# OpenMendel/MendelIHT.jl

Hardware: NVIDIA B200
Metric: iht_iterations_per_sec (higher is better)
Workload: dtype f64 (sweep: f32 LUT partials per slab of 640 samples (512 without the ternary copy), f64 across slabs; top-k candidates re-scored in f64)

## Files before the change

mendeliht.jl_b200/csrc/lut_common.cuh:

```cuda
#pragma once
#include "common.cuh"
#include <cuda_fp16.h>

namespace ihtb {

constexpr int LUT_TABLE_BYTES = 131072;

__device__ __forceinline__ uint32_t smem_u32(const void* p) { return (uint32_t)__cvta_generic_to_shared(p); }
__device__ __forceinline__ void mbar_init(uint32_t bar, uint32_t count) {
    asm volatile("mbarrier.init.shared::cta.b64 [%0], %1;" ::"r"(bar), "r"(count));
}
__device__ __forceinline__ void mbar_arrive(uint32_t bar) {
    asm volatile("mbarrier.arrive.shared::cta.b64 _, [%0];" ::"r"(bar) : "memory");
}
__device__ __forceinline__ void mbar_expect_tx(uint32_t bar, uint32_t bytes) {
    asm volatile("mbarrier.arrive.expect_tx.shared::cta.b64 _, [%0], %1;" ::"r"(bar), "r"(bytes) : "memory");
}
__device__ __forceinline__ void mbar_wait(uint32_t bar, uint32_t parity) {
    asm volatile(
        "{\n\t.reg .pred p;\n"
        "W_%=:\n\t"
        "mbarrier.try_wait.parity.shared::cta.b64 p, [%0], %1;\n\t"
        "@!p bra W_%=;\n\t}"
        ::"r"(bar), "r"(parity) : "memory");
}
__device__ __forceinline__ void bulk_g2s(uint32_t dst, const void* src, uint32_t bytes, uint32_t bar) {
    asm volatile("cp.async.bulk.shared::cluster.global.mbarrier::complete_tx::bytes [%0], [%1], %2, [%3];"
                 ::"r"(dst), "l"(src), "r"(bytes), "r"(bar) : "memory");
}
__device__ __forceinline__ float lds_f32(uint32_t addr) {
    float v;
    asm volatile("ld.shared.f32 %0, [%1];" : "=f"(v) : "r"(addr));
    return v;
}
__device__ __forceinline__ uint32_t lds_u32(uint32_t addr) {
    uint32_t v;
    asm volatile("ld.shared.u32 %0, [%1];" : "=r"(v) : "r"(addr));
    return v;
}
__device__ __forceinline__ uint4 lds_u128(uint32_t addr) {
    uint4 v;
    asm volatile("ld.shared.v4.u32 {%0, %1, %2, %3}, [%4];" : "=r"(v.x), "=r"(v.y), "=r"(v.z), "=r"(v.w) : "r"(addr));
    return v;
}
__device__ __forceinline__ void sts_u32(uint32_t addr, uint32_t v) {
    asm volatile("st.shared.u32 [%0], %1;" ::"r"(addr), "r"(v) : "memory");
}
__device__ __forceinline__ void sts_f32(uint32_t addr, float v) {
    asm volatile("st.shared.f32 [%0], %1;" ::"r"(addr), "f"(v) : "memory");
}
template <int NT>
__device__ __forceinline__ void consumer_bar() {
    asm volatile("bar.sync 1, %0;" ::"n"(NT) : "memory");
}

template <int NT>
__device__ __forceinline__ void lut_build(uint32_t tab, const double* __restrict__ v, double vbar, int64_t n,
                                          int64_t slab, int tid) {
    constexpr int PARTS = NT / 128;
    constexpr int V3_PER = 4 / PARTS;
    const int group = tid & 127, part = tid >> 7;
    const int t = group >> 5, w = group & 31;
    float u[4];
#pragma unroll
    for (int s = 0; s < 4; ++s) {
        int64_t i = slab * 512 + 16 * w + 4 * t + s;
        u[s] = (i < n) ? __double2float_rn(__dsub_rn(v[i], vbar)) : 0.0f;
    }
    auto f = [&](int s, int code) -> float { return code == 2 ? u[s] : (code == 3 ? u[s] + u[s] : 0.0f); };
    const uint32_t rowbase = tab + (uint32_t)(t >> 1) * 65536u + (uint32_t)(t & 1) * 128u + 4u * (uint32_t)w;
#pragma unroll
    for (int c3 = 0; c3 < V3_PER; ++c3) {
        const int v3 = part * V3_PER + c3;
        const float a3 = (v3 == 2) ? u[3] : ((v3 == 3) ? u[3] + u[3] : 0.0f);
        const uint32_t base3 = rowbase + (uint32_t)v3 * (64u * 256u);
#pragma unroll
        for (int v2 = 0; v2 < 4; ++v2) {
            const float a2 = a3 + f(2, v2);
#pragma unroll
            for (int v1 = 0; v1 < 4; ++v1) {
                const float a1 = a2 + f(1, v1);
#pragma unroll
                for (int v0 = 0; v0 < 4; ++v0)
                    sts_f32(base3 + (uint32_t)(v2 << 4 | v1 << 2 | v0) * 256u, a1 + f(0, v0));
            }
        }
    }
}

template <int NT>
__device__ __forceinline__ void lut_build_tern(uint32_t tab, const double* __restrict__ v, double vbar, int64_t n,
                                               int64_t slab, int tid) {
    static_assert(NT == 512, "ternary tables are built by 512 threads");
    const int group = tid & 127, d4 = tid >> 7;
    if (d4 > 2) return;
    const int t = group >> 5, w = group & 31;
    float u[5];
#pragma unroll
    for (int s = 0; s < 5; ++s) {
        int64_t i = slab * 640 + 20 * w + 5 * t + s;
        u[s] = (i < n) ? __double2float_rn(__dsub_rn(v[i], vbar)) : 0.0f;
    }
    auto f = [&](int s, int d) -> float { return d == 1 ? u[s] : (d == 2 ? u[s] + u[s] : 0.0f); };
    const uint32_t rowbase = tab + (uint32_t)(t >> 1) * 65536u + (uint32_t)(t & 1) * 128u + 4u * (uint32_t)w;
    const float a4 = (d4 == 1) ? u[4] : ((d4 == 2) ? u[4] + u[4] : 0.0f);
    const uint32_t base4 = rowbase + (uint32_t)d4 * (81u * 256u);
#pragma unroll
    for (int d3 = 0; d3 < 3; ++d3) {
        const float a3 = a4 + f(3, d3);
#pragma unroll
        for (int d2 = 0; d2 < 3; ++d2) {
            const float a2 = a3 + f(2, d2);
#pragma unroll
            for (int d1 = 0; d1 < 3; ++d1) {
                const float a1 = a2 + f(1, d1);
#pragma unroll
                for (int d0 = 0; d0 < 3; ++d0)
                    sts_f32(base4 + (uint32_t)(27 * d3 + 9 * d2 + 3 * d1 + d0) * 256u, a1 + f(0, d0));
            }
        }
    }
}

__device__ __forceinline__ void lut_build_h2_tern(uint32_t tab, const double* __restrict__ v0, const double* __restrict__ v1,
                                                  double vbar0, double vbar1, float sc0, float sc1, int64_t n, int64_t slab,
                                                  int tid) {
    const int group = tid & 127, d4 = tid >> 7;
    if (d4 > 2) return;
    const int t = group >> 5, w = group & 31;
    float a[5], b[5];
#pragma unroll
    for (int s = 0; s < 5; ++s) {
        int64_t i = slab * 640 + 20 * w + 5 * t + s;
        const float x0 = (i < n) ? __double2float_rn(__dsub_rn(v0[i], vbar0)) * sc0 : 0.0f;
        const float x1 = (i < n) ? __double2float_rn(__dsub_rn(v1[i], vbar1)) * sc1 : 0.0f;
        a[s] = (w & 16) ? x1 : x0;
        b[s] = (w & 16) ? x0 : x1;
    }
    auto fa = [&](int s, int d) -> float { return d == 1 ? a[s] : (d == 2 ? a[s] + a[s] : 0.0f); };
    auto fb = [&](int s, int d) -> float { return d == 1 ? b[s] : (d == 2 ? b[s] + b[s] : 0.0f); };
    const uint32_t rowbase = tab + (uint32_t)(t >> 1) * 65536u + (uint32_t)(t & 1) * 128u + 4u * (uint32_t)w;
    const float a4 = fa(4, d4), b4 = fb(4, d4);
    const uint32_t base4 = rowbase + (uint32_t)d4 * (81u * 256u);
#pragma unroll
    for (int d3 = 0; d3 < 3; ++d3) {
        const float a3 = a4 + fa(3, d3), b3 = b4 + fb(3, d3);
#pragma unroll
        for (int d2 = 0; d2 < 3; ++d2) {
            const float a2 = a3 + fa(2, d2), b2 = b3 + fb(2, d2);
#pragma unroll
            for (int d1 = 0; d1 < 3; ++d1) {
                const float a1 = a2 + fa(1, d1), b1 = b2 + fb(1, d1);
#pragma unroll
                for (int d0 = 0; d0 < 3; ++d0) {
                    const __half2 h = __floats2half2_rn(a1 + fa(0, d0), b1 + fb(0, d0));
                    sts_u32(base4 + (uint32_t)(27 * d3 + 9 * d2 + 3 * d1 + d0) * 256u, *reinterpret_cast<const uint32_t*>(&h));
                }
            }
        }
    }
}

__device__ __forceinline__ void lut_build_h2(uint32_t tab, const double* __restrict__ v0, const double* __restrict__ v1,
                                             double vbar0, double vbar1, float sc0, float sc1, int64_t n, int64_t slab,
                                             int tid) {
    const int group = tid & 127, part = tid >> 7;
    const int t = group >> 5, w = group & 31;
    float a[4], b[4];
#pragma unroll
    for (int s = 0; s < 4; ++s) {
        int64_t i = slab * 512 + 16 * w + 4 * t + s;
        a[s] = (i < n) ? __double2float_rn(__dsub_rn(v0[i], vbar0)) * sc0 : 0.0f;
        b[s] = (i < n) ? __double2float_rn(__dsub_rn(v1[i], vbar1)) * sc1 : 0.0f;
    }
    auto fa = [&](int s, int code) -> float { return code == 2 ? a[s] : (code == 3 ? a[s] + a[s] : 0.0f); };
    auto fb = [&](int s, int code) -> float { return code == 2 ? b[s] : (code == 3 ? b[s] + b[s] : 0.0f); };
    const uint32_t rowbase = tab + (uint32_t)(t >> 1) * 65536u + (uint32_t)(t & 1) * 128u + 4u * (uint32_t)w;
    const int v3 = part;
    const float a3 = fa(3, v3), b3 = fb(3, v3);
    const uint32_t base3 = rowbase + (uint32_t)v3 * (64u * 256u);
#pragma unroll
    for (int v2 = 0; v2 < 4; ++v2) {
        const float a2 = a3 + fa(2, v2), b2 = b3 + fb(2, v2);
#pragma unroll
        for (int v1c = 0; v1c < 4; ++v1c) {
            const float a1 = a2 + fa(1, v1c), b1 = b2 + fb(1, v1c);
#pragma unroll
            for (int v0c = 0; v0c < 4; ++v0c) {
                const __half2 h = __floats2half2_rn(a1 + fa(0, v0c), b1 + fb(0, v0c));
                sts_u32(base3 + (uint32_t)(v2 << 4 | v1c << 2 | v0c) * 256u, *reinterpret_cast<const uint32_t*>(&h));
            }
        }
    }
}

}
```

mendeliht.jl_b200/csrc/sweep_lut.cu:

```cuda
#include "lut_common.cuh"
#include <stdlib.h>

namespace ihtb {

constexpr int LUT_STAGE_COLS = 128;
constexpr int LUT_STAGE_BYTES = LUT_STAGE_COLS * 128;
constexpr int LUT_MAX_STAGES = 8;
constexpr int LUT_SMEM_BYTES = 232448;

struct LutPlan {
    uint32_t bar_full, bar_empty;
    uint32_t tab;
    uint32_t lo0, hi0;
    int n_lo, n_stages;
    __device__ __forceinline__ uint32_t stage(int s) const {
        return (s < n_lo) ? lo0 + (uint32_t)s * LUT_STAGE_BYTES : hi0 + (uint32_t)(s - n_lo) * LUT_STAGE_BYTES;
    }
};
__device__ __forceinline__ LutPlan lut_plan(uint32_t base, uint32_t bytes) {
    LutPlan pl;
    uint32_t end = base + bytes;
    pl.tab = (base + 65535u) & ~65535u;
    pl.bar_full = 0; pl.bar_empty = 0; pl.n_stages = 0;
    uint32_t lo = (base + 127u) & ~127u, lo_end = pl.tab;
    uint32_t hi = pl.tab + LUT_TABLE_BYTES, hi_end = end;
    if (lo + 256u <= lo_end) { pl.bar_full = lo; lo += 256u; }
    else { pl.bar_full = hi; hi += 256u; }
    pl.bar_empty = pl.bar_full + 8u * 2u * LUT_MAX_STAGES;
    pl.lo0 = lo; pl.hi0 = hi;
    pl.n_lo = (lo_end > lo) ? (int)((lo_end - lo) / LUT_STAGE_BYTES) : 0;
    if (pl.n_lo > LUT_MAX_STAGES) pl.n_lo = LUT_MAX_STAGES;
    int n_hi = (hi_end > hi) ? (int)((hi_end - hi) / LUT_STAGE_BYTES) : 0;
    pl.n_stages = pl.n_lo + n_hi;
    if (pl.n_stages > LUT_MAX_STAGES) pl.n_stages = LUT_MAX_STAGES;
    return pl;
}

template <int CW, int G, bool QUAD, bool H2, bool TERN>
__global__ void __launch_bounds__((CW + 1) * 32, 1)
k_sweep_lut(const uint8_t* __restrict__ bed, int64_t cs_j, int64_t cs_s, int64_t p, int64_t p_out, int64_t n,
            int64_t n_slabs, const double* __restrict__ v, const double* __restrict__ v1,
            const double* __restrict__ vbar_p, const float* __restrict__ scale_p, float* __restrict__ part,
            uint32_t dyn_bytes) {
    const double vbar = vbar_p[0];
    const double vbar1 = H2 ? vbar_p[1] : 0.0;
    const float sc0 = H2 ? scale_p[0] : 1.0f, sc1 = H2 ? scale_p[1] : 1.0f;
    constexpr int WPG = CW / G;
    constexpr int CPW = LUT_STAGE_COLS / WPG;
    static_assert(!QUAD || CPW % 4 == 0, "quad layout: a warp owns whole quads");
    static_assert(!H2 || (CW == 16 && CPW == 16), "pair sweep: 512 table builders, 16 columns per warp");
    static_assert(!TERN || (QUAD && CPW == 16), "ternary tiles: quad layout, 16 columns per warp");
    extern __shared__ __align__(128) uint8_t smem_raw[];
    const LutPlan pl = lut_plan(smem_u32(smem_raw), dyn_bytes);
    const int warp = threadIdx.x >> 5, lane = threadIdx.x & 31;
    const int S = pl.n_stages;
    const int period = (S % G == 0) ? S : S * G;

    const int64_t n_cblocks = (p + LUT_STAGE_COLS - 1) / LUT_STAGE_COLS;
    const int64_t units = n_slabs * n_cblocks;
    const int64_t u_beg = units * (int64_t)blockIdx.x / gridDim.x;
    const int64_t u_end = units * (int64_t)(blockIdx.x + 1) / gridDim.x;
    if (u_beg >= u_end) return;
    const int64_t slab_beg = u_beg / n_cblocks, slab_end = (u_end - 1) / n_cblocks;
    const int ncb = (int)n_cblocks;

    if (threadIdx.x == 0) {
        for (int s = 0; s < S; ++s) {
            for (int g = 0; g < G; ++g) mbar_init(pl.bar_full + 8u * (g * LUT_MAX_STAGES + s), 1);
            mbar_init(pl.bar_empty + 8u * s, WPG);
        }
        asm volatile("fence.mbarrier_init.release.cluster;" ::: "memory");
    }
    __syncthreads();

    if (warp == CW) {
        int st = 0; uint32_t ph = 0;
        int grp_of = 0;
        for (int64_t slab = slab_beg; slab <= slab_end; ++slab) {
            const int cb0 = (slab == slab_beg) ? (int)(u_beg - slab * n_cblocks) : 0;
            const int cb1 = (slab == slab_end) ? (int)(u_end - slab * n_cblocks) : ncb;
            for (int cb = cb0; cb < cb1; ++cb) {
                const int64_t j0 = (int64_t)cb * LUT_STAGE_COLS;
                const int ncols = (int)((p - j0 < LUT_STAGE_COLS) ? (p - j0) : LUT_STAGE_COLS);
                const uint32_t fullbar = pl.bar_full + 8u * (uint32_t)(grp_of * LUT_MAX_STAGES + st);
                mbar_wait(pl.bar_empty + 8u * st, ph ^ 1u);
                const uint8_t* src = bed + j0 * cs_j + slab * cs_s;
                if (cs_j == 128) {
                    if (lane == 0) {
                        mbar_expect_tx(fullbar, (uint32_t)ncols * 128u);
                        bulk_g2s(pl.stage(st), src, (uint32_t)ncols * 128u, fullbar);
                    }
                } else {
                    if (lane == 0) mbar_expect_tx(fullbar, (uint32_t)ncols * 128u);
                    __syncwarp();
                    for (int c = lane; c < ncols; c += 32)
                        bulk_g2s(pl.stage(st) + 128u * c, src + (int64_t)c * cs_j, 128u, fullbar);
                }
                if (++st == S) { st = 0; ph ^= 1u; }
                if (++grp_of == G) grp_of = 0;
            }
        }
    } else {
        const int tid = threadIdx.x;
        const int grp = warp / WPG, wg = warp % WPG;
        uint32_t lb[4];
#pragma unroll
        for (int t = 0; t < 4; ++t)
            lb[t] = pl.tab + (uint32_t)(t >> 1) * 65536u + (uint32_t)(t & 1) * 128u + 4u * (uint32_t)lane;
        constexpr int NACC = H2 ? 2 * CPW : CPW;
        constexpr int LPC = 32 / NACC > 0 ? 32 / NACC : 1;
        const int vidx = TERN ? (lane & (NACC - 1)) : lane / LPC;
        const int col = wg * CPW + vidx % CPW;
        const bool writer = TERN ? (lane < NACC) : (lane & (LPC - 1)) == 0;
        const uint32_t lqs = TERN ? ((((uint32_t)lane >> 2) & 3u) << 9) : 0u;
        const uint32_t lane_off = (uint32_t)(wg * CPW) * 128u + (QUAD ? 16u : 4u) * (uint32_t)lane;
        int st = grp % S, ip = grp % period; uint32_t ph = (uint32_t)((grp / period) & 1);
        const uint32_t my_full = pl.bar_full + 8u * (uint32_t)(grp * LUT_MAX_STAGES);
        int i_next = grp;
        int i_base = 0;
        for (int64_t slab = slab_beg; slab <= slab_end; ++slab) {
            const int cb0 = (slab == slab_beg) ? (int)(u_beg - slab * n_cblocks) : 0;
            const int cb1 = (slab == slab_end) ? (int)(u_end - slab * n_cblocks) : ncb;
            consumer_bar<CW * 32>();
            if (H2 && TERN) lut_build_h2_tern(pl.tab, v, v1, vbar, vbar1, sc0, sc1, n, slab, tid);
            else if (H2) lut_build_h2(pl.tab, v, v1, vbar, vbar1, sc0, sc1, n, slab, tid);
            else if (TERN) lut_build_tern<CW * 32>(pl.tab, v, vbar, n, slab, tid);
            else lut_build<CW * 32>(pl.tab, v, vbar, n, slab, tid);
            consumer_bar<CW * 32>();
            float* __restrict__ outp = part + ((int64_t)(H2 ? vidx / CPW : 0) * n_slabs + slab) * p_out + col;
            const int i_end = i_base + (cb1 - cb0);
            for (; i_next < i_end; i_next += G) {
                const int cb = cb0 + (i_next - i_base);
                mbar_wait(my_full + 8u * st, ph);
                const uint32_t colbase = pl.stage(st) + lane_off;
                float acc[NACC];
                uint4 q4 = make_uint4(0u, 0u, 0u, 0u);
#pragma unroll
                for (int c = 0; c < CPW; ++c) {
                    uint32_t w;
                    if (QUAD) {
                        if ((c & 3) == 0) q4 = lds_u128(colbase + ((512u * (c >> 2)) ^ lqs));
                        w = (c & 3) == 0 ? q4.x : (c & 3) == 1 ? q4.y : (c & 3) == 2 ? q4.z : q4.w;
                    } else {
                        w = lds_u32(colbase + 128u * c);
                    }
                    if (!H2) {
                        const float t0 = lds_f32(__byte_perm(w, lb[0], 0x7604));
                        const float t1 = lds_f32(__byte_perm(w, lb[1], 0x7614));
                        const float t2 = lds_f32(__byte_perm(w, lb[2], 0x7624));
                        const float t3 = lds_f32(__byte_perm(w, lb[3], 0x7634));
                        acc[c] = (t0 + t1) + (t2 + t3);
                    } else {
                        const uint32_t r0 = lds_u32(__byte_perm(w, lb[0], 0x7604));
                        const uint32_t r1 = lds_u32(__byte_perm(w, lb[1], 0x7614));
                        const uint32_t r2 = lds_u32(__byte_perm(w, lb[2], 0x7624));
                        const uint32_t r3 = lds_u32(__byte_perm(w, lb[3], 0x7634));
                        const __half2 h = __hadd2(__hadd2(*reinterpret_cast<const __half2*>(&r0), *reinterpret_cast<const __half2*>(&r1)),
                                                  __hadd2(*reinterpret_cast<const __half2*>(&r2), *reinterpret_cast<const __half2*>(&r3)));
                        const float2 f = __half22float2(h);
                        acc[c] = f.x;
                        acc[(H2 ? CPW : 0) + c] = f.y;
                    }
                }
                __syncwarp();
                if (lane == 0) mbar_arrive(pl.bar_empty + 8u * st);
                if (TERN) {
                    int o = NACC / 2;
#pragma unroll
                    for (int h = NACC / 2; h >= 1; h >>= 1, o >>= 1) {
#pragma unroll
                        for (int c = 0; c < h; ++c) acc[c] = acc[c] + __shfl_xor_sync(0xffffffffu, acc[c + h], o);
                    }
#pragma unroll
                    for (int oo = 16; oo >= NACC; oo >>= 1) acc[0] += __shfl_xor_sync(0xffffffffu, acc[0], oo);
                } else {
                    int o = 16;
#pragma unroll
                    for (int h = NACC / 2; h >= 1; h >>= 1, o >>= 1) {
                        const bool upper = (lane & o) != 0;
#pragma unroll
                        for (int c = 0; c < h; ++c) {
                            const float send = upper ? acc[c] : acc[c + h];
                            const float keep = upper ? acc[c + h] : acc[c];
                            acc[c] = keep + __shfl_xor_sync(0xffffffffu, send, o);
                        }
                    }
#pragma unroll
                    for (int oo = 16 / NACC; oo >= 1; oo >>= 1) acc[0] += __shfl_xor_sync(0xffffffffu, acc[0], oo);
                }
                const int jj = cb * LUT_STAGE_COLS + col;
                if (writer && jj < (int)p_out) outp[cb * LUT_STAGE_COLS] = acc[0];
                st += G; if (st >= S) st -= S;
                ip += G; if (ip >= period) { ip -= period; ph ^= 1u; }
            }
            i_base = i_end;
        }
    }
}

bool sweep_tmem_enabled(const ihtb_geno* g);
bool sweep_uses_tern(const ihtb_geno* g) { return g->tern.p != nullptr && g->quad && !sweep_tmem_enabled(g); }
int64_t sweep_fast_num_slabs(const ihtb_geno* g) { return sweep_uses_tern(g) ? g->tern_slabs : g->stride / 128; }

bool sweep_tmem_enabled(const ihtb_geno* g);
void sweep_tmem_partials(const ihtb_geno* g, const double* d_v, const double* d_vbar, float* d_part, cudaStream_t s);
void sweep_tmem_pair_partials(const ihtb_geno* g, const double* d_v0, const double* d_v1, const double* d_vbar,
                              const float* d_scale, float* d_part, cudaStream_t s);

template <bool QUAD, bool H2, bool TERN = false>
static void launch_lut(const ihtb_geno* g, const double* d_v, const double* d_v1, const double* d_vbar,
                       const float* d_scale, float* d_part, cudaStream_t s) {
    ensure_dynamic_smem(k_sweep_lut<16, 2, QUAD, H2, TERN>, LUT_SMEM_BYTES);
    const int64_t n_slabs = TERN ? g->tern_slabs : g->stride / 128;
    const int64_t n_cblocks = ceil_div(g->p4, LUT_STAGE_COLS);
    int64_t units = n_slabs * n_cblocks;
    int grid = g->sm_count;
    if (units < grid) grid = (int)units;
    IHTB_CHECK(g->p < (int64_t(1) << 31) - 256, IHTB_EDIM, "more than 2^31 SNP columns on one GPU");
    IHTB_LAUNCH((k_sweep_lut<16, 2, QUAD, H2, TERN>), grid, 17 * 32, LUT_SMEM_BYTES, s, TERN ? g->tern.p : g->bed.p, g->cs_j,
                g->cs_s, g->p4, g->p, g->n, n_slabs, d_v, d_v1, d_vbar, d_scale, d_part, (uint32_t)LUT_SMEM_BYTES);
}

void sweep_fast_partials(const ihtb_geno* g, const double* d_v, const double* d_vbar, float* d_part, int64_t* n_slabs_out,
                         cudaStream_t s) {
    if (n_slabs_out) *n_slabs_out = sweep_fast_num_slabs(g);
    if (sweep_tmem_enabled(g)) { sweep_tmem_partials(g, d_v, d_vbar, d_part, s); return; }
    if (sweep_uses_tern(g)) launch_lut<true, false, true>(g, d_v, nullptr, d_vbar, nullptr, d_part, s);
    else if (g->quad) launch_lut<true, false>(g, d_v, nullptr, d_vbar, nullptr, d_part, s);
    else launch_lut<false, false>(g, d_v, nullptr, d_vbar, nullptr, d_part, s);
}

void sweep_fast_kernel_only(const ihtb_geno* g, const double* d_v, const double* d_vbar, float* d_part, cudaStream_t s) {
    sweep_fast_partials(g, d_v, d_vbar, d_part, nullptr, s);
}

void sweep_pair_partials(const ihtb_geno* g, const double* d_v0, const double* d_v1, const double* d_vbar,
                         const float* d_scale, float* d_part, cudaStream_t s) {
    IHTB_CHECK(g->cs_j == 128, IHTB_EUNSUPPORTED, "the pair sweep needs a tiled layout");
    if (sweep_tmem_enabled(g)) { sweep_tmem_pair_partials(g, d_v0, d_v1, d_vbar, d_scale, d_part, s); return; }
    if (sweep_uses_tern(g)) launch_lut<true, true, true>(g, d_v0, d_v1, d_vbar, d_scale, d_part, s);
    else if (g->quad) launch_lut<true, true>(g, d_v0, d_v1, d_vbar, d_scale, d_part, s);
    else launch_lut<false, true>(g, d_v0, d_v1, d_vbar, d_scale, d_part, s);
}

}
```

Measured before the change: 837.7.

## Use one-column-per-lane ternary LUT sweep with four consumer groups

For the ternary (non-pair) sweep, each lane now owns a single column. It reads 32 words with swizzled addresses, builds the table indices with prmt against a packed base, and sums in registers. This removes the cross-lane shuffle reduction. The consumer group count rises from 2 to 4 for this path, so the barrier block is enlarged, stage buffers are aligned to 512 bytes, and the period and stage wraparound are generalised to a non-divisible stage count. The change raises register pressure (32 words plus 32 partial sums per lane) and risks bank conflicts if the swizzle does not match the tile layout.

```diff
diff --git a/mendeliht.jl_b200/csrc/lut_common.cuh b/mendeliht.jl_b200/csrc/lut_common.cuh
--- a/mendeliht.jl_b200/csrc/lut_common.cuh
+++ b/mendeliht.jl_b200/csrc/lut_common.cuh
@@ -43,6 +43,12 @@
     asm volatile("ld.shared.v4.u32 {%0, %1, %2, %3}, [%4];" : "=r"(v.x), "=r"(v.y), "=r"(v.z), "=r"(v.w) : "r"(addr));
     return v;
 }
+template <uint32_t SEL>
+__device__ __forceinline__ uint32_t prmt(uint32_t a, uint32_t b) {
+    uint32_t d;
+    asm("prmt.b32 %0, %1, %2, %3;" : "=r"(d) : "r"(a), "r"(b), "n"(SEL));
+    return d;
+}
 __device__ __forceinline__ void sts_u32(uint32_t addr, uint32_t v) {
     asm volatile("st.shared.u32 [%0], %1;" ::"r"(addr), "r"(v) : "memory");
 }
diff --git a/mendeliht.jl_b200/csrc/sweep_lut.cu b/mendeliht.jl_b200/csrc/sweep_lut.cu
--- a/mendeliht.jl_b200/csrc/sweep_lut.cu
+++ b/mendeliht.jl_b200/csrc/sweep_lut.cu
@@ -6,6 +6,8 @@
 constexpr int LUT_STAGE_COLS = 128;
 constexpr int LUT_STAGE_BYTES = LUT_STAGE_COLS * 128;
 constexpr int LUT_MAX_STAGES = 8;
+constexpr int LUT_MAX_GROUPS = 4;
+constexpr uint32_t LUT_BAR_BYTES = 8u * (LUT_MAX_GROUPS + 1) * LUT_MAX_STAGES;
 constexpr int LUT_SMEM_BYTES = 232448;
 
 struct LutPlan {
@@ -24,9 +26,10 @@
     pl.bar_full = 0; pl.bar_empty = 0; pl.n_stages = 0;
     uint32_t lo = (base + 127u) & ~127u, lo_end = pl.tab;
     uint32_t hi = pl.tab + LUT_TABLE_BYTES, hi_end = end;
-    if (lo + 256u <= lo_end) { pl.bar_full = lo; lo += 256u; }
-    else { pl.bar_full = hi; hi += 256u; }
-    pl.bar_empty = pl.bar_full + 8u * 2u * LUT_MAX_STAGES;
+    if (lo + LUT_BAR_BYTES <= lo_end) { pl.bar_full = lo; lo += LUT_BAR_BYTES; }
+    else { pl.bar_full = hi; hi += LUT_BAR_BYTES; }
+    pl.bar_empty = pl.bar_full + 8u * LUT_MAX_GROUPS * LUT_MAX_STAGES;
+    lo = (lo + 511u) & ~511u; hi = (hi + 511u) & ~511u;
     pl.lo0 = lo; pl.hi0 = hi;
     pl.n_lo = (lo_end > lo) ? (int)((lo_end - lo) / LUT_STAGE_BYTES) : 0;
     if (pl.n_lo > LUT_MAX_STAGES) pl.n_lo = LUT_MAX_STAGES;
@@ -45,16 +48,20 @@
     const double vbar = vbar_p[0];
     const double vbar1 = H2 ? vbar_p[1] : 0.0;
     const float sc0 = H2 ? scale_p[0] : 1.0f, sc1 = H2 ? scale_p[1] : 1.0f;
+    constexpr bool COL = TERN && !H2;
     constexpr int WPG = CW / G;
     constexpr int CPW = LUT_STAGE_COLS / WPG;
+    static_assert(G <= LUT_MAX_GROUPS, "barrier block holds LUT_MAX_GROUPS full barriers per stage");
     static_assert(!QUAD || CPW % 4 == 0, "quad layout: a warp owns whole quads");
     static_assert(!H2 || (CW == 16 && CPW == 16), "pair sweep: 512 table builders, 16 columns per warp");
-    static_assert(!TERN || (QUAD && CPW == 16), "ternary tiles: quad layout, 16 columns per warp");
+    static_assert(!TERN || (QUAD && CW == 16), "ternary tiles: quad layout, 512 table builders");
+    static_assert(!COL || CPW == 32, "one column per lane: 32 columns per warp");
     extern __shared__ __align__(128) uint8_t smem_raw[];
     const LutPlan pl = lut_plan(smem_u32(smem_raw), dyn_bytes);
     const int warp = threadIdx.x >> 5, lane = threadIdx.x & 31;
     const int S = pl.n_stages;
-    const int period = (S % G == 0) ? S : S * G;
+    int period = S;
+    while (period % G != 0) period += S;
 
     const int64_t n_cblocks = (p + LUT_STAGE_COLS - 1) / LUT_STAGE_COLS;
     const int64_t units = n_slabs * n_cblocks;
@@ -114,6 +121,10 @@
         const bool writer = TERN ? (lane < NACC) : (lane & (LPC - 1)) == 0;
         const uint32_t lqs = TERN ? ((((uint32_t)lane >> 2) & 3u) << 9) : 0u;
         const uint32_t lane_off = (uint32_t)(wg * CPW) * 128u + (QUAD ? 16u : 4u) * (uint32_t)lane;
+        const uint32_t w0 = 8u * ((uint32_t)lane & 3u) + ((uint32_t)lane >> 2);
+        const uint32_t col_off = (uint32_t)(wg * CPW) * 128u + ((uint32_t)lane >> 2) * 512u + 16u * w0 +
+                                 4u * (((uint32_t)lane & 3u) ^ (w0 & 3u));
+        const uint32_t y0 = 4u * w0 | (128u + 4u * w0) << 8 | (pl.tab >> 16) << 16 | ((pl.tab >> 16) + 1u) << 24;
         int st = grp % S, ip = grp % period; uint32_t ph = (uint32_t)((grp / period) & 1);
         const uint32_t my_full = pl.bar_full + 8u * (uint32_t)(grp * LUT_MAX_STAGES);
         int i_next = grp;
@@ -132,65 +143,93 @@
             for (; i_next < i_end; i_next += G) {
                 const int cb = cb0 + (i_next - i_base);
                 mbar_wait(my_full + 8u * st, ph);
-                const uint32_t colbase = pl.stage(st) + lane_off;
-                float acc[NACC];
-                uint4 q4 = make_uint4(0u, 0u, 0u, 0u);
-#pragma unroll
-                for (int c = 0; c < CPW; ++c) {
-                    uint32_t w;
-                    if (QUAD) {
-                        if ((c & 3) == 0) q4 = lds_u128(colbase + ((512u * (c >> 2)) ^ lqs));
-                        w = (c & 3) == 0 ? q4.x : (c & 3) == 1 ? q4.y : (c & 3) == 2 ? q4.z : q4.w;
+                float sum;
+                if constexpr (COL) {
+                    const uint32_t a0 = pl.stage(st) + col_off;
+                    uint32_t wd[32];
+#pragma unroll
+                    for (int s = 0; s < 32; ++s) wd[s] = lds_u32(a0 ^ (16u * s + 4u * (s & 3)));
+                    __syncwarp();
+                    if (lane == 0) mbar_arrive(pl.bar_empty + 8u * st);
+                    float ws[32];
+#pragma unroll
+                    for (int s = 0; s < 32; ++s) {
+                        const uint32_t y = y0 ^ (uint32_t)(4 * s * 0x0101);
+                        const float t0 = lds_f32(prmt<0xE604u>(wd[s], y));
+                        const float t1 = lds_f32(prmt<0xE615u>(wd[s], y));
+                        const float t2 = lds_f32(prmt<0xF724u>(wd[s], y));
+                        const float t3 = lds_f32(prmt<0xF735u>(wd[s], y));
+                        ws[s] = (t0 + t1) + (t2 + t3);
+                    }
+#pragma unroll
+                    for (int k = 0, done = 0; k < 5; ++k) {
+                        const int b = (k < 4) ? (8 >> k) : 16;
+#pragma unroll
+                        for (int s = 0; s < 32; ++s)
+                            if ((s & (done | b)) == 0) ws[s] = ws[s] + ws[s | b];
+                        done |= b;
+                    }
+                    sum = ws[0];
+                } else {
+                    const uint32_t colbase = pl.stage(st) + lane_off;
+                    float acc[NACC];
+                    uint4 q4 = make_uint4(0u, 0u, 0u, 0u);
+#pragma unroll
+                    for (int c = 0; c < CPW; ++c) {
+                        uint32_t w;
+                        if (QUAD) {
+                            if ((c & 3) == 0) q4 = lds_u128(colbase + ((512u * (c >> 2)) ^ lqs));
+                            w = (c & 3) == 0 ? q4.x : (c & 3) == 1 ? q4.y : (c & 3) == 2 ? q4.z : q4.w;
+                        } else {
+                            w = lds_u32(colbase + 128u * c);
+                        }
+                        if (!H2) {
+                            const float t0 = lds_f32(__byte_perm(w, lb[0], 0x7604));
+                            const float t1 = lds_f32(__byte_perm(w, lb[1], 0x7614));
+                            const float t2 = lds_f32(__byte_perm(w, lb[2], 0x7624));
+                            const float t3 = lds_f32(__byte_perm(w, lb[3], 0x7634));
+                            acc[c] = (t0 + t1) + (t2 + t3);
+                        } else {
+                            const uint32_t r0 = lds_u32(__byte_perm(w, lb[0], 0x7604));
+                            const uint32_t r1 = lds_u32(__byte_perm(w, lb[1], 0x7614));
+                            const uint32_t r2 = lds_u32(__byte_perm(w, lb[2], 0x7624));
+                            const uint32_t r3 = lds_u32(__byte_perm(w, lb[3], 0x7634));
+                            const __half2 h = __hadd2(__hadd2(*reinterpret_cast<const __half2*>(&r0), *reinterpret_cast<const __half2*>(&r1)),
+                                                      __hadd2(*reinterpret_cast<const __half2*>(&r2), *reinterpret_cast<const __half2*>(&r3)));
+                            const float2 f = __half22float2(h);
+                            acc[c] = f.x;
+                            acc[(H2 ? CPW : 0) + c] = f.y;
+                        }
+                    }
+                    __syncwarp();
+                    if (lane == 0) mbar_arrive(pl.bar_empty + 8u * st);
+                    if (TERN) {
+                        int o = NACC / 2;
+#pragma unroll
+                        for (int h = NACC / 2; h >= 1; h >>= 1, o >>= 1) {
+#pragma unroll
+                            for (int c = 0; c < h; ++c) acc[c] = acc[c] + __shfl_xor_sync(0xffffffffu, acc[c + h], o);
+                        }
                     } else {
-                        w = lds_u32(colbase + 128u * c);
-                    }
-                    if (!H2) {
-                        const float t0 = lds_f32(__byte_perm(w, lb[0], 0x7604));
-                        const float t1 = lds_f32(__byte_perm(w, lb[1], 0x7614));
-                        const float t2 = lds_f32(__byte_perm(w, lb[2], 0x7624));
-                        const float t3 = lds_f32(__byte_perm(w, lb[3], 0x7634));
-                        acc[c] = (t0 + t1) + (t2 + t3);
-                    } else {
-                        const uint32_t r0 = lds_u32(__byte_perm(w, lb[0], 0x7604));
-                        const uint32_t r1 = lds_u32(__byte_perm(w, lb[1], 0x7614));
-                        const uint32_t r2 = lds_u32(__byte_perm(w, lb[2], 0x7624));
-                        const uint32_t r3 = lds_u32(__byte_perm(w, lb[3], 0x7634));
-                        const __half2 h = __hadd2(__hadd2(*reinterpret_cast<const __half2*>(&r0), *reinterpret_cast<const __half2*>(&r1)),
-                                                  __hadd2(*reinterpret_cast<const __half2*>(&r2), *reinterpret_cast<const __half2*>(&r3)));
-                        const float2 f = __half22float2(h);
-                        acc[c] = f.x;
-                        acc[(H2 ? CPW : 0) + c] = f.y;
-                    }
-                }
-                __syncwarp();
-                if (lane == 0) mbar_arrive(pl.bar_empty + 8u * st);
-                if (TERN) {
-                    int o = NACC / 2;
-#pragma unroll
-                    for (int h = NACC / 2; h >= 1; h >>= 1, o >>= 1) {
-#pragma unroll
-                        for (int c = 0; c < h; ++c) acc[c] = acc[c] + __shfl_xor_sync(0xffffffffu, acc[c + h], o);
-                    }
-#pragma unroll
-                    for (int oo = 16; oo >= NACC; oo >>= 1) acc[0] += __shfl_xor_sync(0xffffffffu, acc[0], oo);
-                } else {
-                    int o = 16;
-#pragma unroll
-                    for (int h = NACC / 2; h >= 1; h >>= 1, o >>= 1) {
-                        const bool upper = (lane & o) != 0;
-#pragma unroll
-                        for (int c = 0; c < h; ++c) {
-                            const float send = upper ? acc[c] : acc[c + h];
-                            const float keep = upper ? acc[c + h] : acc[c];
-                            acc[c] = keep + __shfl_xor_sync(0xffffffffu, send, o);
-                        }
-                    }
-#pragma unroll
-                    for (int oo = 16 / NACC; oo >= 1; oo >>= 1) acc[0] += __shfl_xor_sync(0xffffffffu, acc[0], oo);
+                        int o = 16;
+#pragma unroll
+                        for (int h = NACC / 2; h >= 1; h >>= 1, o >>= 1) {
+                            const bool upper = (lane & o) != 0;
+#pragma unroll
+                            for (int c = 0; c < h; ++c) {
+                                const float send = upper ? acc[c] : acc[c + h];
+                                const float keep = upper ? acc[c + h] : acc[c];
+                                acc[c] = keep + __shfl_xor_sync(0xffffffffu, send, o);
+                            }
+                        }
+#pragma unroll
+                        for (int oo = 16 / NACC; oo >= 1; oo >>= 1) acc[0] += __shfl_xor_sync(0xffffffffu, acc[0], oo);
+                    }
+                    sum = acc[0];
                 }
                 const int jj = cb * LUT_STAGE_COLS + col;
-                if (writer && jj < (int)p_out) outp[cb * LUT_STAGE_COLS] = acc[0];
-                st += G; if (st >= S) st -= S;
+                if (writer && jj < (int)p_out) outp[cb * LUT_STAGE_COLS] = sum;
+                st += G; while (st >= S) st -= S;
                 ip += G; if (ip >= period) { ip -= period; ph ^= 1u; }
             }
             i_base = i_end;
@@ -210,14 +249,15 @@
 template <bool QUAD, bool H2, bool TERN = false>
 static void launch_lut(const ihtb_geno* g, const double* d_v, const double* d_v1, const double* d_vbar,
                        const float* d_scale, float* d_part, cudaStream_t s) {
-    ensure_dynamic_smem(k_sweep_lut<16, 2, QUAD, H2, TERN>, LUT_SMEM_BYTES);
+    constexpr int G = (TERN && !H2) ? 4 : 2;
+    ensure_dynamic_smem(k_sweep_lut<16, G, QUAD, H2, TERN>, LUT_SMEM_BYTES);
     const int64_t n_slabs = TERN ? g->tern_slabs : g->stride / 128;
     const int64_t n_cblocks = ceil_div(g->p4, LUT_STAGE_COLS);
     int64_t units = n_slabs * n_cblocks;
     int grid = g->sm_count;
     if (units < grid) grid = (int)units;
     IHTB_CHECK(g->p < (int64_t(1) << 31) - 256, IHTB_EDIM, "more than 2^31 SNP columns on one GPU");
-    IHTB_LAUNCH((k_sweep_lut<16, 2, QUAD, H2, TERN>), grid, 17 * 32, LUT_SMEM_BYTES, s, TERN ? g->tern.p : g->bed.p, g->cs_j,
+    IHTB_LAUNCH((k_sweep_lut<16, G, QUAD, H2, TERN>), grid, 17 * 32, LUT_SMEM_BYTES, s, TERN ? g->tern.p : g->bed.p, g->cs_j,
                 g->cs_s, g->p4, g->p, g->n, n_slabs, d_v, d_v1, d_vbar, d_scale, d_part, (uint32_t)LUT_SMEM_BYTES);
 }
 
```

Measured after the change: 924.3 (median of 6 runs). 1.1x the previous value.
